# bharath5673/StrongSORT-YOLO

Measured on AMD Instinct MI355X. Metric: tracked frames/sec (whole node), 1280x720@30det, higher is better.
Workload: dtype f32 association / f64 Kalman+LSAP (f16 detector convs, fp32 ReID network on own v_mfma_f32 kernels)

## Files before the change

### strongsort_yolo_amd/csrc/ss_ops.hip

```cpp
#include <hip/hip_fp16.h>
#include <hip/hip_runtime.h>
#include <stdint.h>
#include <stdlib.h>
#include <string>
#include "../../include/strongsort_hip.h"

struct NvEntry { void* stream; const int* n; int batch; };
static thread_local NvEntry g_nv[8] = {};
static inline const int* nv_for(void* stream, long long batch)
{
    for (const NvEntry& e : g_nv) if (e.n && e.stream == stream && e.batch == batch) return e.n;
    return nullptr;
}
static inline int nv_batch(void* stream)
{
    for (const NvEntry& e : g_nv) if (e.n && e.stream == stream) return e.batch;
    return 0;
}

static int g_opt_pw_epilogue = 1, g_opt_pw_splitk = 1, g_opt_osnet_chains = 1;

typedef _Float16 h8 __attribute__((ext_vector_type(8)));
typedef _Float16 h4 __attribute__((ext_vector_type(4)));
typedef float f4 __attribute__((ext_vector_type(4)));

__device__ inline float act_apply(float v, int act)
{
    if (act == 1) return v > 0.f ? v : 0.f;
    if (act == 2) return v * __builtin_amdgcn_rcpf(1.0f + __expf(-v));
    if (act == 3) return __builtin_amdgcn_rcpf(1.0f + __expf(-v));
    return v;
}

__global__ __launch_bounds__(256) void k_bias_act8(__half* __restrict__ x, const __half* __restrict__ bias,
                                                  const __half* __restrict__ res, size_t n_vec, int C8, int act)
{
    for (size_t i = blockIdx.x * (size_t)blockDim.x + threadIdx.x; i < n_vec; i += (size_t)gridDim.x * blockDim.x) {
        h8 v = reinterpret_cast<h8*>(x)[i];
        h8 b = reinterpret_cast<const h8*>(bias)[i % C8];
        h8 r;
        if (res) r = reinterpret_cast<const h8*>(res)[i];
#pragma unroll
        for (int k = 0; k < 8; ++k) {
            float f = (float)v[k] + (float)b[k];
            if (res) f += (float)r[k];
            v[k] = (_Float16)act_apply(f, act);
        }
        reinterpret_cast<h8*>(x)[i] = v;
    }
}

__global__ __launch_bounds__(256) void k_bias_act1(__half* __restrict__ x, const __half* __restrict__ bias,
                                                  const __half* __restrict__ res, size_t n, int C, int act)
{
    for (size_t i = blockIdx.x * (size_t)blockDim.x + threadIdx.x; i < n; i += (size_t)gridDim.x * blockDim.x) {
        float f = __half2float(x[i]) + __half2float(bias[i % C]);
        if (res) f += __half2float(res[i]);
        x[i] = __float2half(act_apply(f, act));
    }
}

__device__ __forceinline__ float ss_mix_lo(unsigned a, unsigned b, float c)
{ float d; asm("v_fma_mix_f32 %0, %1, %2, %3 op_sel:[0,0,0] op_sel_hi:[1,1,0]" : "=v"(d) : "v"(a), "v"(b), "v"(c)); return d; }
__device__ __forceinline__ float ss_mix_hi(unsigned a, unsigned b, float c)
{ float d; asm("v_fma_mix_f32 %0, %1, %2, %3 op_sel:[1,1,0] op_sel_hi:[1,1,0]" : "=v"(d) : "v"(a), "v"(b), "v"(c)); return d; }
__device__ __forceinline__ void ss_dw_tap8(const h8& v, const h8& w, float (&acc)[8])
{
    const uint4 vu = __builtin_bit_cast(uint4, v), wu = __builtin_bit_cast(uint4, w);
    acc[0] = ss_mix_lo(vu.x, wu.x, acc[0]); acc[1] = ss_mix_hi(vu.x, wu.x, acc[1]);
    acc[2] = ss_mix_lo(vu.y, wu.y, acc[2]); acc[3] = ss_mix_hi(vu.y, wu.y, acc[3]);
    acc[4] = ss_mix_lo(vu.z, wu.z, acc[4]); acc[5] = ss_mix_hi(vu.z, wu.z, acc[5]);
    acc[6] = ss_mix_lo(vu.w, wu.w, acc[6]); acc[7] = ss_mix_hi(vu.w, wu.w, acc[7]);
}

__global__ __launch_bounds__(256) void k_dw3x3(const __half* __restrict__ x, const __half* __restrict__ w9,
                                              const __half* __restrict__ bias, __half* __restrict__ y, int N, int H,
                                              int W, int C8, int act)
{
    const size_t total = (size_t)N * H * W * C8;
    for (size_t i = blockIdx.x * (size_t)blockDim.x + threadIdx.x; i < total; i += (size_t)gridDim.x * blockDim.x) {
        const int c8 = (int)(i % C8);
        const size_t p = i / C8;
        const int w = (int)(p % W), h = (int)((p / W) % H);
        const size_t nb = (p / ((size_t)W * H)) * H;
        float acc[8];
        {
            h8 b = reinterpret_cast<const h8*>(bias)[c8];
#pragma unroll
            for (int k = 0; k < 8; ++k) acc[k] = (float)b[k];
        }
#pragma unroll
        for (int dy = -1; dy <= 1; ++dy) {
            const int hh = h + dy;
            if (hh < 0 || hh >= H) continue;
#pragma unroll
            for (int dx = -1; dx <= 1; ++dx) {
                const int ww = w + dx;
                if (ww < 0 || ww >= W) continue;
                h8 v = reinterpret_cast<const h8*>(x)[((nb + hh) * W + ww) * C8 + c8];
                h8 k9 = reinterpret_cast<const h8*>(w9)[((dy + 1) * 3 + dx + 1) * C8 + c8];
                ss_dw_tap8(v, k9, acc);
            }
        }
// ... 332 lines not shown
    f4 acc[MT];
#pragma unroll
    for (int mt = 0; mt < MT; ++mt) acc[mt] = f4{ 0.f, 0.f, 0.f, 0.f };
    h8 a[MT][2], b[2], an[MT][2], bn[2];
    int kc = wave * KC;
    if (kc < K) { load_a(kc, a); load_b(kc, b); }
    for (; kc < K; kc += 4 * KC) {
        const bool more = kc + 4 * KC < K;
        if (more) { load_a(kc + 4 * KC, an); load_b(kc + 4 * KC, bn); }
#pragma unroll
        for (int ks = 0; ks < 2; ++ks) {
            if (kc + ks * 32 >= K) break;
#pragma unroll
            for (int mt = 0; mt < MT; ++mt) acc[mt] = __builtin_amdgcn_mfma_f32_16x16x32_f16(a[mt][ks], b[ks], acc[mt], 0, 0, 0);
        }
        if (more) {
#pragma unroll
            for (int mt = 0; mt < MT; ++mt) { a[mt][0] = an[mt][0]; a[mt][1] = an[mt][1]; }
            b[0] = bn[0]; b[1] = bn[1];
        }
    }
#pragma unroll
    for (int mt = 0; mt < MT; ++mt)
#pragma unroll
        for (int j = 0; j < 4; ++j) Red[(wave * BN + mt * 16 + 4 * q + j) * RP + n] = acc[mt][j];
    __syncthreads();
    constexpr int CG = BN / 8;
    if (tid < 16 * CG) {
        const int row = tid / CG, cg = tid - row * CG;
        const size_t p = (size_t)bx * 16 + row;
        const int oc = n0 + cg * 8;
        if (p < (size_t)M && oc < N) {
            const h8 bb = *reinterpret_cast<const h8*>(bias + oc);
            h8 r = z8;
            if (res) r = *reinterpret_cast<const h8*>(res + p * N + oc);
            h8 o;
#pragma unroll
            for (int j = 0; j < 8; ++j) {
                const int ch = cg * 8 + j;
                const float sum = ((Red[(0 * BN + ch) * RP + row] + Red[(1 * BN + ch) * RP + row]) + Red[(2 * BN + ch) * RP + row]) +
                                  Red[(3 * BN + ch) * RP + row];
                float f = (float)(_Float16)sum + (float)bb[j];
                if (res && !res_after) f += (float)r[j];
                f = act_apply(f, act);
                if (res && res_after) f = (float)(_Float16)f + (float)r[j];
                o[j] = (_Float16)f;
            }
            *reinterpret_cast<h8*>(out + p * out_ld + oc) = o;
            if (out2 && oc >= c0 && oc < c0 + cn) *reinterpret_cast<h8*>(out2 + p * cn + (oc - c0)) = o;
        }
    }
}

template <int BN, bool CONV3>
__global__ __launch_bounds__(256) void k_pw_splitk(PwArgs A) { pw_splitk_body<BN, CONV3>(A, blockIdx.x, blockIdx.y); }

#define PW_GROUP_MAX 12
struct PwGroup { PwArgs p[PW_GROUP_MAX]; int start[PW_GROUP_MAX + 1]; int form[PW_GROUP_MAX]; int n; };

#ifndef SS_GRP_WAVES
#define SS_GRP_WAVES 6
#endif
template <int BN, bool CONV3, bool SPLITK>
__global__ __launch_bounds__(256)
__attribute__((amdgpu_waves_per_eu(SPLITK || !SS_GRP_WAVES ? 1 : SS_GRP_WAVES)))
void k_pw_group(PwGroup G)
{
    __shared__ __attribute__((aligned(16))) _Float16 pw_lds[pw_lds_halfs<BN, 1, true>()];
    int bx = blockIdx.x, p = 0;
    for (int i = 1; i < G.n; ++i) if (bx >= G.start[i]) p = i;
    bx -= G.start[p];
    const int form = G.form[p];
    if constexpr (SPLITK) { if (form == 1) { pw_splitk_body<BN, CONV3>(G.p[p], bx, 0); return; } }
    if (BN == 80 && G.p[p].N <= 64) pw_body<64, 1, CONV3, true>(G.p[p], bx, 0, pw_lds);
    else pw_body<BN, 1, CONV3, true>(G.p[p], bx, 0, pw_lds);
}

struct BnArgs {
    const __half* x; const __half* w1; const __half* b1; const __half* w2; const __half* b2;
    __half* out; int out_ld; __half* out2;
    int B, H, W, add, TW, TH, tiles_x, tiles_y;
};

template <int CI, int CO, int PT>
__device__ __forceinline__ void bn_conv(const _Float16* __restrict__ In, const int (&pbase)[PT], const int* __restrict__ tapoff,
                                        const __half* __restrict__ w, _Float16* __restrict__ Ws, f4 (&acc)[CO / 16][PT], const int tid)
{
    constexpr int C = CI;
    constexpr int MT = CO / 16, WP = 72, K = 9 * CI, WV = (CO * 8 + 255) / 256;
    const int lane = tid & 63, q = lane >> 4, n = lane & 15;
    const h8 z8 = { 0, 0, 0, 0, 0, 0, 0, 0 };
    auto load_w = [&](int k0, h8 (&wr)[WV]) {
#pragma unroll
        for (int j = 0; j < WV; ++j) {
            const int i = tid + j * 256, r = i >> 3, c8 = i & 7, kk = k0 + c8 * 8;
            wr[j] = (i < CO * 8 && kk < K) ? *reinterpret_cast<const h8*>(w + (size_t)r * K + kk) : z8;
        }
    };
    h8 wr[WV], wn[WV];
    load_w(0, wr);
    int buf = 0;
    for (int k0 = 0; k0 < K; k0 += 64, buf ^= 1) {
        _Float16* wb = Ws + buf * (CO * WP);
#pragma unroll
        for (int j = 0; j < WV; ++j) {
            const int i = tid + j * 256, r = i >> 3, c8 = i & 7;
            if (i < CO * 8) *reinterpret_cast<h8*>(wb + r * WP + c8 * 8) = wr[j];
        }
        if (k0 + 64 < K) load_w(k0 + 64, wn);
        __syncthreads();
        h8 b[2][PT], a[2][MT];
#pragma unroll
        for (int ks = 0; ks < 2; ++ks) {
            const int kk = k0 + ks * 32 + 8 * q, tap = kk / C, c = kk % C;
            const bool kv = kk < K;
            const int boff = kv ? tapoff[tap] + c : 0;
#pragma unroll
            for (int pt = 0; pt < PT; ++pt) {
                b[ks][pt] = *reinterpret_cast<const h8*>(In + pbase[pt] + boff);
                if (!kv) b[ks][pt] = z8;
            }
#pragma unroll
            for (int mt = 0; mt < MT; ++mt) a[ks][mt] = *reinterpret_cast<const h8*>(wb + (mt * 16 + n) * WP + ks * 32 + 8 * q);
        }
#pragma unroll
        for (int ks = 0; ks < 2; ++ks) {
            if (k0 + ks * 32 >= K) break;
#pragma unroll
            for (int mt = 0; mt < MT; ++mt)
#pragma unroll
                for (int pt = 0; pt < PT; ++pt)
                    acc[mt][pt] = __builtin_amdgcn_mfma_f32_16x16x32_f16(a[ks][mt], b[ks][pt], acc[mt][pt], 0, 0, 0);
        }
        if (k0 + 64 < K) {
#pragma unroll
            for (int j = 0; j < WV; ++j) wr[j] = wn[j];
        }
    }
}

template <int C, int PT1, int PT2>
__global__ __launch_bounds__(256) __attribute__((amdgpu_waves_per_eu(!SS_TAIL_BUMP ? 1 : C == 16 ? 6 : 1))) void k_bneck(BnArgs A)
{
    extern __shared__ __attribute__((aligned(16))) char bn_smem[];
    constexpr int MT = C / 16, P = C + 8, WP = 72;
    const int tid = threadIdx.x, lane = tid & 63, wave = tid >> 6, q = lane >> 4, n = lane & 15;
    const int TW = A.TW, TH = A.TH, XW = TW + 4, XH = TH + 4, RW = TW + 2, RH = TH + 2;
    _Float16* Xs = reinterpret_cast<_Float16*>(bn_smem);
    _Float16* Ts = Xs + XH * XW * P;
    _Float16* Ws = Ts + ((RH * RW * P + 7) & ~7);
    int* tap1 = reinterpret_cast<int*>(Ws + 2 * C * WP);
    int* tap2 = tap1 + 16;
    const int tpi = A.tiles_x * A.tiles_y;
    const int img = blockIdx.x / tpi, trm = blockIdx.x - img * tpi, tyi = trm / A.tiles_x, txi = trm - tyi * A.tiles_x;
    const int oy0 = tyi * TH, ox0 = txi * TW, H = A.H, W = A.W;
    const h8 z8 = { 0, 0, 0, 0, 0, 0, 0, 0 };
    if (tid < 9) { const int ky = tid / 3, kx = tid - ky * 3; tap1[tid] = (ky * XW + kx) * P; tap2[tid] = (ky * RW + kx) * P; }
    const __half* xi = A.x + (size_t)img * H * W * C;
    constexpr int VPC = C / 8;
    const int rowv = XW * VPC;
    for (int r = wave; r < XH; r += 4) {
        const int iy = oy0 - 2 + r;
        const bool rok = iy >= 0 && iy < H;
        const __half* src = xi + (size_t)(rok ? iy : 0) * W * C;
        _Float16* dst = Xs + r * XW * P;
        for (int i0 = lane; i0 < rowv; i0 += 512) {
            h8 tmp[8];
#pragma unroll
            for (int u = 0; u < 8; ++u) {
                const int i = i0 + 64 * u, c = i / VPC, v = i % VPC, ix = ox0 - 2 + c;
                const bool ok = rok && i < rowv && ix >= 0 && ix < W;
                tmp[u] = ok ? *reinterpret_cast<const h8*>(src + (size_t)ix * C + v * 8) : z8;
            }
#pragma unroll
            for (int u = 0; u < 8; ++u) {
                const int i = i0 + 64 * u, c = i / VPC, v = i % VPC;
                if (i < rowv) *reinterpret_cast<h8*>(dst + c * P + v * 8) = tmp[u];
            }
        }
    }
    {
        int pb[PT1], tpix[PT1];
        bool inimg[PT1];
#pragma unroll
        for (int pt = 0; pt < PT1; ++pt) {
            const int p = (wave * PT1 + pt) * 16 + n;
            int ry = p / RW, rx = p - ry * RW;
            const bool ok = p < RH * RW;
            if (!ok) { ry = 0; rx = 0; }
            const int iy = oy0 - 1 + ry, ix = ox0 - 1 + rx;
            inimg[pt] = ok && iy >= 0 && iy < H && ix >= 0 && ix < W;
            tpix[pt] = ok ? p : -1;
            pb[pt] = (ry * XW + rx) * P;
        }
        f4 acc[MT][PT1];
#pragma unroll
        for (int mt = 0; mt < MT; ++mt)
#pragma unroll
            for (int pt = 0; pt < PT1; ++pt) acc[mt][pt] = f4{ 0.f, 0.f, 0.f, 0.f };
        bn_conv<C, C, PT1>(Xs, pb, tap1, A.w1, Ws, acc, tid);
#pragma unroll
        for (int mt = 0; mt < MT; ++mt) {
            const h4 bb = *reinterpret_cast<const h4*>(A.b1 + mt * 16 + 4 * q);
#pragma unroll
            for (int pt = 0; pt < PT1; ++pt) {
                if (tpix[pt] < 0) continue;
                h4 o;
#pragma unroll
                for (int j = 0; j < 4; ++j) {
                    float f = act_apply((float)(_Float16)acc[mt][pt][j] + (float)bb[j], 2);
                    asm volatile("" : "+v"(f));
                    o[j] = inimg[pt] ? (_Float16)f : (_Float16)0.f;
                }
                *reinterpret_cast<h4*>(Ts + tpix[pt] * P + mt * 16 + 4 * q) = o;
            }
        }
    }
    __syncthreads();
    {
        int pb[PT2], opix[PT2], xoff[PT2];
#pragma unroll
        for (int pt = 0; pt < PT2; ++pt) {
            const int p = (wave * PT2 + pt) * 16 + n;
            int ty = p / TW, tx = p - ty * TW;
            const bool ok = p < TH * TW && oy0 + ty < H && ox0 + tx < W;
            if (!ok) { ty = 0; tx = 0; }
            pb[pt] = (ty * RW + tx) * P;
            xoff[pt] = ((ty + 2) * XW + tx + 2) * P;
            opix[pt] = ok ? (img * H + oy0 + ty) * W + ox0 + tx : -1;
        }
        f4 acc[MT][PT2];
#pragma unroll
        for (int mt = 0; mt < MT; ++mt)
#pragma unroll
            for (int pt = 0; pt < PT2; ++pt) acc[mt][pt] = f4{ 0.f, 0.f, 0.f, 0.f };
        bn_conv<C, C, PT2>(Ts, pb, tap2, A.w2, Ws, acc, tid);
#pragma unroll
        for (int mt = 0; mt < MT; ++mt) {
            const h4 bb = *reinterpret_cast<const h4*>(A.b2 + mt * 16 + 4 * q);
#pragma unroll
            for (int pt = 0; pt < PT2; ++pt) {
                if (opix[pt] < 0) continue;
                const h4 xr = *reinterpret_cast<const h4*>(Xs + xoff[pt] + mt * 16 + 4 * q);
                h4 o;
#pragma unroll
                for (int j = 0; j < 4; ++j) {
                    float f = act_apply((float)(_Float16)acc[mt][pt][j] + (float)bb[j], 2);
                    asm volatile("" : "+v"(f));
                    if (A.add) f = (float)(_Float16)f + (float)xr[j];
                    o[j] = (_Float16)f;
                }
                *reinterpret_cast<h4*>(A.out + (size_t)opix[pt] * A.out_ld + mt * 16 + 4 * q) = o;
                if (A.out2) *reinterpret_cast<h4*>(A.out2 + (size_t)opix[pt] * C + mt * 16 + 4 * q) = o;
            }
        }
    }
}

struct HeadArgs {
    const __half* x;
    const __half* w1[2]; const __half* b1[2]; const __half* w2[2]; const __half* b2[2]; const __half* w3[2]; const __half* b3[2];
    __half* out[2]; int nout[2];
    int B, H, W, TW, TH, tiles_x, tiles_y;
};

template <int CI, int CM, int PT1, int PT2>
__device__ __forceinline__ void head_body(const HeadArgs& A, const int br, char* smem)
{
    constexpr int MT = CM / 16, PX = CI + 8, PM = CM + 8, WP = 72, KB3 = (CM + 31) / 32;
    const int tid = threadIdx.x, lane = tid & 63, wave = tid >> 6, q = lane >> 4, n = lane & 15;
    const int TW = A.TW, TH = A.TH, XW = TW + 4, XH = TH + 4, RW = TW + 2, RH = TH + 2;
    _Float16* Xs = reinterpret_cast<_Float16*>(smem);
    _Float16* Ts = Xs + ((XH * XW * PX + 7) & ~7);
    _Float16* Ws = Ts + ((RH * RW * PM + 7) & ~7);
    int* tap1 = reinterpret_cast<int*>(Ws + 2 * 80 * WP);
    int* tap2 = tap1 + 16;
    _Float16* Us = Xs;
    const int tpi = A.tiles_x * A.tiles_y;
    const int img = blockIdx.x / tpi, trm = blockIdx.x - img * tpi, tyi = trm / A.tiles_x, txi = trm - tyi * A.tiles_x;
    const int oy0 = tyi * TH, ox0 = txi * TW, H = A.H, W = A.W;
    const h8 z8 = { 0, 0, 0, 0, 0, 0, 0, 0 };
    if (tid < 9) { const int ky = tid / 3, kx = tid - ky * 3; tap1[tid] = (ky * XW + kx) * PX; tap2[tid] = (ky * RW + kx) * PM; }
    const __half* xi = A.x + (size_t)img * H * W * CI;
    constexpr int VPC = CI / 8;
    const int rowv = XW * VPC;
    for (int r = wave; r < XH; r += 4) {
        const int iy = oy0 - 2 + r;
        const bool rok = iy >= 0 && iy < H;
        const __half* src = xi + (size_t)(rok ? iy : 0) * W * CI;
        _Float16* dst = Xs + r * XW * PX;
        for (int i0 = lane; i0 < rowv; i0 += 512) {
            h8 tmp[8];
#pragma unroll
            for (int u = 0; u < 8; ++u) {
                const int i = i0 + 64 * u, c = i / VPC, v = i % VPC, ix = ox0 - 2 + c;
                const bool ok = rok && i < rowv && ix >= 0 && ix < W;
                tmp[u] = ok ? *reinterpret_cast<const h8*>(src + (size_t)ix * CI + v * 8) : z8;
            }
#pragma unroll
            for (int u = 0; u < 8; ++u) {
                const int i = i0 + 64 * u, c = i / VPC, v = i % VPC;
                if (i < rowv) *reinterpret_cast<h8*>(dst + c * PX + v * 8) = tmp[u];
            }
        }
    }
    {
        int pb[PT1], tpix[PT1];
        bool inimg[PT1];
#pragma unroll
        for (int pt = 0; pt < PT1; ++pt) {
            const int p = (wave * PT1 + pt) * 16 + n;
            int ry = p / RW, rx = p - ry * RW;
            const bool ok = p < RH * RW;
            if (!ok) { ry = 0; rx = 0; }
            const int iy = oy0 - 1 + ry, ix = ox0 - 1 + rx;
            inimg[pt] = ok && iy >= 0 && iy < H && ix >= 0 && ix < W;
            tpix[pt] = ok ? p : -1;
            pb[pt] = (ry * XW + rx) * PX;
        }
        f4 acc[MT][PT1];
#pragma unroll
        for (int mt = 0; mt < MT; ++mt)
#pragma unroll
            for (int pt = 0; pt < PT1; ++pt) acc[mt][pt] = f4{ 0.f, 0.f, 0.f, 0.f };
        bn_conv<CI, CM, PT1>(Xs, pb, tap1, A.w1[br], Ws, acc, tid);
#pragma unroll
        for (int mt = 0; mt < MT; ++mt) {
            const h4 bb = *reinterpret_cast<const h4*>(A.b1[br] + mt * 16 + 4 * q);
#pragma unroll
            for (int pt = 0; pt < PT1; ++pt) {
                if (tpix[pt] < 0) continue;
                h4 o;
#pragma unroll
                for (int j = 0; j < 4; ++j) {
                    float f = act_apply((float)(_Float16)acc[mt][pt][j] + (float)bb[j], 2);
                    asm volatile("" : "+v"(f));
                    o[j] = inimg[pt] ? (_Float16)f : (_Float16)0.f;
                }
// ... 1761 lines not shown
        if (c.N > nmax) nmax = c.N;
        order[i] = i;
        cost[i] = (long long)c.ksize * c.ksize * c.Cin;
    }
    for (int i = 1; i < n; ++i)
        for (int j = i; j > 0 && cost[order[j]] > cost[order[j - 1]]; --j) { const int t = order[j]; order[j] = order[j - 1]; order[j - 1] = t; }
    int wgs = 0;
    for (int s = 0; s < n; ++s) {
        const ss_conv_desc& c = d[order[s]];
        ConvGeom g{ c.H, c.W, c.Cin, (c.H - 1) / c.stride + 1, (c.W - 1) / c.stride + 1, c.stride };
        const long long M = (long long)c.B * g.OH * g.OW;
        if (M > 0x7fffffffLL) return SS_ERR_INVALID;
        const int K = c.ksize * c.ksize * c.Cin;
        G.p[s] = PwArgs{ (const __half*)c.x, (const __half*)c.w, (const __half*)c.bias, nullptr, (int)M, K, c.N, c.act, 0, (__half*)c.out,
                         c.N, nullptr, 0, 0, g, nullptr, 0 };
        G.form[s] = (splitk_allowed && conv3 && K >= 512 && M <= 4096) ? 1 : 0;
        G.start[s] = wgs;
        wgs += (int)(G.form[s] == 1 ? (M + 15) / 16 : (M + 63) / 64);
    }
    for (int s = n; s < PW_GROUP_MAX; ++s) { G.p[s] = G.p[0]; G.form[s] = 0; G.start[s] = wgs; }
    G.start[PW_GROUP_MAX] = wgs;
    G.n = n;
    hipStream_t st = (hipStream_t)stream;
    bool any_splitk = false;
    for (int s = 0; s < n; ++s) any_splitk = any_splitk || G.form[s] == 1;
#define SS_GRP(BN) do { if (conv3 && any_splitk) hipLaunchKernelGGL((k_pw_group<BN, true, true>), dim3(wgs), dim3(256), 0, st, G);            \
                        else if (conv3) hipLaunchKernelGGL((k_pw_group<BN, true, false>), dim3(wgs), dim3(256), 0, st, G);                    \
                        else hipLaunchKernelGGL((k_pw_group<BN, false, false>), dim3(wgs), dim3(256), 0, st, G); } while (0)
    if (nmax <= 32) SS_GRP(32);
    else if (nmax <= 64) SS_GRP(64);
    else SS_GRP(80);
#undef SS_GRP
    return hipGetLastError() == hipSuccess ? SS_OK : SS_ERR_HIP;
}

extern "C" int ss_op_upcat_f16(void* stream, const void* lo, const void* hi, void* out, int B, int h, int w, int C1, int C2, int lo_first)
{
    if (!lo || !hi || !out || B < 1 || h < 1 || w < 1 || C1 < 8 || C1 % 8 || C2 < 8 || C2 % 8) return SS_ERR_INVALID;
    const size_t total = (size_t)B * 4 * h * w * ((C1 + C2) / 8);
    hipLaunchKernelGGL(k_upcat, dim3(grid_for(total, 256)), dim3(256), 0, (hipStream_t)stream, (const __half*)lo, (const __half*)hi,
                       (__half*)out, B, h, w, C1 / 8, C2 / 8, lo_first);
    return hipGetLastError() == hipSuccess ? SS_OK : SS_ERR_HIP;
}

extern "C" int ss_op_osnet_head_f16(void* stream, const void* x, const void* w, const void* bias, void* out, int N, int HW, int C, int F)
{
    if (!x || !w || !bias || !out || N < 1 || HW < 1 || C != 128 || F < 1) return SS_ERR_INVALID;
    hipLaunchKernelGGL(k_osnet_head<128>, dim3((N + 3) / 4), dim3(256), 0, (hipStream_t)stream, (const __half*)x, (const __half*)w,
                       (const __half*)bias, (__half*)out, N, HW, F, nv_for(stream, N));
    return hipGetLastError() == hipSuccess ? SS_OK : SS_ERR_HIP;
}

extern "C" int ss_op_psa_attention_f16(void* stream, const void* qkv, const void* pe, void* out, int B, int N, int heads, float scale)
{
    if (!qkv || !out || B < 1 || B > 65535 || N < 1 || N > 16 * PSA_MAXT || heads < 1 || heads > 64) return SS_ERR_INVALID;
    const int NP = (N + 31) & ~31;
    hipLaunchKernelGGL(k_psa_attn, dim3((N + 63) / 64, heads, B), dim3(256), (size_t)64 * (NP + 16) * 2, (hipStream_t)stream,
                       (const __half*)qkv, (const __half*)pe, (__half*)out, N, heads, scale);
    return hipGetLastError() == hipSuccess ? SS_OK : SS_ERR_HIP;
}

extern "C" int ss_op_sppf_pools_f16(void* stream, const void* x, void* out, int B, int H, int W, int C)
{
    if (!x || !out || B < 1 || H < 1 || W < 1 || C < 8 || C % 8 || H * W > 1024) return SS_ERR_INVALID;
    hipLaunchKernelGGL(k_sppf_pools, dim3((unsigned)(B * (C / 8))), dim3(256), (size_t)2 * H * W * 16, (hipStream_t)stream,
                       (const __half*)x, (__half*)out, H, W, C / 8);
    return hipGetLastError() == hipSuccess ? SS_OK : SS_ERR_HIP;
}

extern "C" int ss_op_conv0_f16(void* stream, const void* x, const void* w_prep, const void* bias, void* y, int B, int H, int W, int Cout,
                               int act)
{
    if (!x || !w_prep || !bias || !y || B < 1 || H < 2 || W < 128 || W % 128 || (W * 3) % 8 || (Cout != 16 && Cout != 32 && Cout != 48))
        return SS_ERR_INVALID;
    const int OH = (H - 1) / 2 + 1;
    const dim3 grid(W / 128, (OH + C0_ROWS - 1) / C0_ROWS, B), block(256);
    hipStream_t st = (hipStream_t)stream;
#define SS_C0(CO) hipLaunchKernelGGL(k_conv0<CO>, grid, block, 0, st, (const __half*)x, (const __half*)w_prep, (const __half*)bias, (__half*)y, H, W, act)
    if (Cout == 16) SS_C0(16); else if (Cout == 32) SS_C0(32); else SS_C0(48);
#undef SS_C0
    return hipGetLastError() == hipSuccess ? SS_OK : SS_ERR_HIP;
}

extern "C" int ss_op_bottleneck_f16(void* stream, const void* x, const void* w1, const void* b1, const void* w2, const void* b2, int B, int H,
                                    int W, int C, int add, void* out, int out_ld, void* out2)
{
    if (!x || !w1 || !b1 || !w2 || !b2 || !out || B < 1 || H < 1 || W < 1 || (C != 16 && C != 32 && C != 64 && C != 128) || out_ld < C || out_ld % 4 ||
        ((uintptr_t)out % 8) || ((uintptr_t)x % 16) || ((uintptr_t)w1 % 16) || ((uintptr_t)w2 % 16) || (out2 && ((uintptr_t)out2 % 8)))
        return SS_ERR_INVALID;
    const long long M = (long long)B * H * W;
    const bool big = M / 128 >= 512 && C <= 64;
    BnArgs A{ (const __half*)x, (const __half*)w1, (const __half*)b1, (const __half*)w2, (const __half*)b2, (__half*)out, out_ld, (__half*)out2,
              B, H, W, add, big ? 16 : 8, 8, 0, 0 };
    A.tiles_x = (W + A.TW - 1) / A.TW; A.tiles_y = (H + A.TH - 1) / A.TH;
    const int P = C + 8;
    const size_t lds = ((size_t)(A.TH + 4) * (A.TW + 4) * P + (((size_t)(A.TH + 2) * (A.TW + 2) * P + 7) & ~(size_t)7) + 2 * (size_t)C * 72) * 2 + 128;
    const dim3 grid((unsigned)(B * A.tiles_x * A.tiles_y));
    hipStream_t st = (hipStream_t)stream;
#define SS_BN(CC, P1, P2) do { static unsigned long long attr = 0; int dv_ = 0; (void)hipGetDevice(&dv_); if (!(attr >> (dv_ & 63) & 1)) { (void)hipFuncSetAttribute((const void*)k_bneck<CC, P1, P2>, hipFuncAttributeMaxDynamicSharedMemorySize, 160 * 1024 - 512); attr |= 1ull << (dv_ & 63); }    \
                               hipLaunchKernelGGL((k_bneck<CC, P1, P2>), grid, dim3(256), lds, st, A); } while (0)
    if (big) { if (C == 16) SS_BN(16, 3, 2); else if (C == 32) SS_BN(32, 3, 2); else SS_BN(64, 3, 2); }
    else { if (C == 16) SS_BN(16, 2, 1); else if (C == 32) SS_BN(32, 2, 1); else if (C == 64) SS_BN(64, 2, 1); else SS_BN(128, 2, 1); }
#undef SS_BN
    return hipGetLastError() == hipSuccess ? SS_OK : SS_ERR_HIP;
}

extern "C" int ss_op_head_f16(void* stream, const void* x, const void* const* w1, const void* const* b1, const void* const* w2,
                              const void* const* b2, const void* const* w3, const void* const* b3, void* const* out, const int* nout,
                              int B, int H, int W, int Cin, int tile16)
{
    if (!x || !w1 || !b1 || !w2 || !b2 || !w3 || !b3 || !out || !nout || B < 1 || H < 1 || W < 1 || (Cin != 64 && Cin != 128 && Cin != 256) ||
        ((uintptr_t)x % 16))
        return SS_ERR_INVALID;
    HeadArgs A;
    A.x = (const __half*)x;
    for (int b = 0; b < 2; ++b) {
        const int cm = b ? 80 : 64;
        if (!w1[b] || !b1[b] || !w2[b] || !b2[b] || !w3[b] || !b3[b] || !out[b] || nout[b] < 8 || nout[b] % 8 || nout[b] > cm ||
            ((uintptr_t)w1[b] % 16) || ((uintptr_t)w2[b] % 16) || ((uintptr_t)w3[b] % 16) || ((uintptr_t)out[b] % 8))
            return SS_ERR_INVALID;
        A.w1[b] = (const __half*)w1[b]; A.b1[b] = (const __half*)b1[b]; A.w2[b] = (const __half*)w2[b]; A.b2[b] = (const __half*)b2[b];
        A.w3[b] = (const __half*)w3[b]; A.b3[b] = (const __half*)b3[b]; A.out[b] = (__half*)out[b]; A.nout[b] = nout[b];
    }
    const bool big = tile16 != 0 && Cin == 64;
    A.B = B; A.H = H; A.W = W; A.TW = big ? 16 : 8; A.TH = 8;
    A.tiles_x = (W + A.TW - 1) / A.TW; A.tiles_y = (H + A.TH - 1) / A.TH;
    const size_t xs = ((size_t)(A.TH + 4) * (A.TW + 4) * (Cin + 8) + 7) & ~(size_t)7, ts = ((size_t)(A.TH + 2) * (A.TW + 2) * 88 + 7) & ~(size_t)7;
    const size_t lds = (xs + ts + 2 * 80 * 72) * 2 + 128;
    if (lds > 160 * 1024 - 512) return SS_ERR_INVALID;
    const dim3 grid((unsigned)(B * A.tiles_x * A.tiles_y), 2);
    hipStream_t st = (hipStream_t)stream;
#define SS_HD(CC, P1, P2) do { static unsigned long long attr = 0; int dv_ = 0; (void)hipGetDevice(&dv_); if (!(attr >> (dv_ & 63) & 1)) { (void)hipFuncSetAttribute((const void*)k_head<CC, P1, P2>, hipFuncAttributeMaxDynamicSharedMemorySize, 160 * 1024 - 512); attr |= 1ull << (dv_ & 63); }    \
                               hipLaunchKernelGGL((k_head<CC, P1, P2>), grid, dim3(256), lds, st, A); } while (0)
    if (big) SS_HD(64, 3, 2);
    else if (Cin == 64) SS_HD(64, 2, 1);
    else if (Cin == 128) SS_HD(128, 2, 1);
    else SS_HD(256, 2, 1);
#undef SS_HD
    return hipGetLastError() == hipSuccess ? SS_OK : SS_ERR_HIP;
}

extern "C" int ss_op_set_valid_images(void* stream, const int* d_n, int batch)
{
    NvEntry* slot = nullptr;
    for (NvEntry& e : g_nv) if (e.n && e.stream == stream) slot = &e;
    if (!d_n) { if (slot) *slot = NvEntry{}; return SS_OK; }
    if (batch < 1) return SS_ERR_INVALID;
    if (!slot) for (NvEntry& e : g_nv) if (!e.n) { slot = &e; break; }
    if (!slot) return SS_ERR_CAPACITY;
    *slot = NvEntry{ stream, d_n, batch };
    return SS_OK;
}

extern int g_opt_jpeg_subseq_words;
int ss_aflink_chunk_option(int value);
extern "C" int ss_op_set_option(const char* name, int value)
{
    if (!name) return SS_ERR_INVALID;
    const std::string n(name);
    if (n == "pw_epilogue") g_opt_pw_epilogue = value;
    else if (n == "pw_splitk") g_opt_pw_splitk = value;
    else if (n == "osnet_chains") g_opt_osnet_chains = value;
    else if (n == "jpeg_subseq_words") { if (value != 4 && value != 8 && value != 16 && value != 32) return SS_ERR_INVALID; g_opt_jpeg_subseq_words = value; }
    else if (n == "aflink_chunk") return ss_aflink_chunk_option(value);
    else return SS_ERR_INVALID;
    return SS_OK;
}
```

Measured before the change: 8615.

## Add persistent bottleneck kernel keeping both conv weights resident in LDS

Result: slower. 8478 (-1.6%).

```diff
diff --git a/strongsort_yolo_amd/csrc/ss_ops.hip b/strongsort_yolo_amd/csrc/ss_ops.hip
--- a/strongsort_yolo_amd/csrc/ss_ops.hip
+++ b/strongsort_yolo_amd/csrc/ss_ops.hip
@@ -19,6 +19,7 @@
 }
 
 static int g_opt_pw_epilogue = 1, g_opt_pw_splitk = 1, g_opt_osnet_chains = 1;
+static int g_opt_bneck_resident = 1;
 
 typedef _Float16 h8 __attribute__((ext_vector_type(8)));
 typedef _Float16 h4 __attribute__((ext_vector_type(4)));
@@ -517,11 +518,41 @@
     int B, H, W, add, TW, TH, tiles_x, tiles_y;
 };
 
+template <int C, int MT, int PT>
+__device__ __forceinline__ void bn_slice(const _Float16* __restrict__ In, const int (&pbase)[PT], const int* __restrict__ tapoff,
+                                         const _Float16* __restrict__ wl, const int wmt, const int k0, const int q, f4 (&acc)[MT][PT])
+{
+    constexpr int K = 9 * C;
+    const h8 z8 = { 0, 0, 0, 0, 0, 0, 0, 0 };
+    h8 b[2][PT], a[2][MT];
+#pragma unroll
+    for (int ks = 0; ks < 2; ++ks) {
+        const int kk = k0 + ks * 32 + 8 * q, tap = kk / C, c = kk % C;
+        const bool kv = kk < K;
+        const int boff = kv ? tapoff[tap] + c : 0;
+#pragma unroll
+        for (int pt = 0; pt < PT; ++pt) {
+            b[ks][pt] = *reinterpret_cast<const h8*>(In + pbase[pt] + boff);
+            if (!kv) b[ks][pt] = z8;
+        }
+#pragma unroll
+        for (int mt = 0; mt < MT; ++mt) a[ks][mt] = *reinterpret_cast<const h8*>(wl + mt * wmt + ks * 32);
+    }
+#pragma unroll
+    for (int ks = 0; ks < 2; ++ks) {
+        if (k0 + ks * 32 >= K) break;
+#pragma unroll
+        for (int mt = 0; mt < MT; ++mt)
+#pragma unroll
+            for (int pt = 0; pt < PT; ++pt)
+                acc[mt][pt] = __builtin_amdgcn_mfma_f32_16x16x32_f16(a[ks][mt], b[ks][pt], acc[mt][pt], 0, 0, 0);
+    }
+}
+
 template <int CI, int CO, int PT>
 __device__ __forceinline__ void bn_conv(const _Float16* __restrict__ In, const int (&pbase)[PT], const int* __restrict__ tapoff,
                                         const __half* __restrict__ w, _Float16* __restrict__ Ws, f4 (&acc)[CO / 16][PT], const int tid)
 {
-    constexpr int C = CI;
     constexpr int MT = CO / 16, WP = 72, K = 9 * CI, WV = (CO * 8 + 255) / 256;
     const int lane = tid & 63, q = lane >> 4, n = lane & 15;
     const h8 z8 = { 0, 0, 0, 0, 0, 0, 0, 0 };
@@ -544,32 +575,59 @@
         }
         if (k0 + 64 < K) load_w(k0 + 64, wn);
         __syncthreads();
-        h8 b[2][PT], a[2][MT];
-#pragma unroll
-        for (int ks = 0; ks < 2; ++ks) {
-            const int kk = k0 + ks * 32 + 8 * q, tap = kk / C, c = kk % C;
-            const bool kv = kk < K;
-            const int boff = kv ? tapoff[tap] + c : 0;
-#pragma unroll
-            for (int pt = 0; pt < PT; ++pt) {
-                b[ks][pt] = *reinterpret_cast<const h8*>(In + pbase[pt] + boff);
-                if (!kv) b[ks][pt] = z8;
-            }
-#pragma unroll
-            for (int mt = 0; mt < MT; ++mt) a[ks][mt] = *reinterpret_cast<const h8*>(wb + (mt * 16 + n) * WP + ks * 32 + 8 * q);
-        }
-#pragma unroll
-        for (int ks = 0; ks < 2; ++ks) {
-            if (k0 + ks * 32 >= K) break;
-#pragma unroll
-            for (int mt = 0; mt < MT; ++mt)
-#pragma unroll
-                for (int pt = 0; pt < PT; ++pt)
-                    acc[mt][pt] = __builtin_amdgcn_mfma_f32_16x16x32_f16(a[ks][mt], b[ks][pt], acc[mt][pt], 0, 0, 0);
-        }
+        bn_slice<CI, MT, PT>(In, pbase, tapoff, wb + n * WP + 8 * q, 16 * WP, k0, q, acc);
         if (k0 + 64 < K) {
 #pragma unroll
             for (int j = 0; j < WV; ++j) wr[j] = wn[j];
+        }
+    }
+}
+
+template <int C, int PT>
+__device__ __forceinline__ void bn_mid_epilogue(const f4 (&acc)[C / 16][PT], const _Float16* __restrict__ bias, const int (&tpix)[PT],
+                                                const bool (&inimg)[PT], _Float16* __restrict__ Ts, const int q)
+{
+    constexpr int MT = C / 16, P = C + 8;
+#pragma unroll
+    for (int mt = 0; mt < MT; ++mt) {
+        const h4 bb = *reinterpret_cast<const h4*>(bias + mt * 16 + 4 * q);
+#pragma unroll
+        for (int pt = 0; pt < PT; ++pt) {
+            if (tpix[pt] < 0) continue;
+            h4 o;
+#pragma unroll
+            for (int j = 0; j < 4; ++j) {
+                float f = act_apply((float)(_Float16)acc[mt][pt][j] + (float)bb[j], 2);
+                asm volatile("" : "+v"(f));
+                o[j] = inimg[pt] ? (_Float16)f : (_Float16)0.f;
+            }
+            *reinterpret_cast<h4*>(Ts + tpix[pt] * P + mt * 16 + 4 * q) = o;
+        }
+    }
+}
+
+template <int C, int PT>
+__device__ __forceinline__ void bn_out_epilogue(const f4 (&acc)[C / 16][PT], const _Float16* __restrict__ bias, const int (&opix)[PT],
+                                                const int (&xoff)[PT], const _Float16* __restrict__ Xs, const BnArgs& A, const int q)
+{
+    constexpr int MT = C / 16;
+#pragma unroll
+    for (int mt = 0; mt < MT; ++mt) {
+        const h4 bb = *reinterpret_cast<const h4*>(bias + mt * 16 + 4 * q);
+#pragma unroll
+        for (int pt = 0; pt < PT; ++pt) {
+            if (opix[pt] < 0) continue;
+            const h4 xr = *reinterpret_cast<const h4*>(Xs + xoff[pt] + mt * 16 + 4 * q);
+            h4 o;
+#pragma unroll
+            for (int j = 0; j < 4; ++j) {
+                float f = act_apply((float)(_Float16)acc[mt][pt][j] + (float)bb[j], 2);
+                asm volatile("" : "+v"(f));
+                if (A.add) f = (float)(_Float16)f + (float)xr[j];
+                o[j] = (_Float16)f;
+            }
+            *reinterpret_cast<h4*>(A.out + (size_t)opix[pt] * A.out_ld + mt * 16 + 4 * q) = o;
+            if (A.out2) *reinterpret_cast<h4*>(A.out2 + (size_t)opix[pt] * C + mt * 16 + 4 * q) = o;
         }
     }
 }
@@ -634,22 +692,7 @@
 #pragma unroll
             for (int pt = 0; pt < PT1; ++pt) acc[mt][pt] = f4{ 0.f, 0.f, 0.f, 0.f };
         bn_conv<C, C, PT1>(Xs, pb, tap1, A.w1, Ws, acc, tid);
-#pragma unroll
-        for (int mt = 0; mt < MT; ++mt) {
-            const h4 bb = *reinterpret_cast<const h4*>(A.b1 + mt * 16 + 4 * q);
-#pragma unroll
-            for (int pt = 0; pt < PT1; ++pt) {
-                if (tpix[pt] < 0) continue;
-                h4 o;
-#pragma unroll
-                for (int j = 0; j < 4; ++j) {
-                    float f = act_apply((float)(_Float16)acc[mt][pt][j] + (float)bb[j], 2);
-                    asm volatile("" : "+v"(f));
-                    o[j] = inimg[pt] ? (_Float16)f : (_Float16)0.f;
-                }
-                *reinterpret_cast<h4*>(Ts + tpix[pt] * P + mt * 16 + 4 * q) = o;
-            }
-        }
+        bn_mid_epilogue<C, PT1>(acc, reinterpret_cast<const _Float16*>(A.b1), tpix, inimg, Ts, q);
     }
     __syncthreads();
     {
@@ -670,25 +713,153 @@
 #pragma unroll
             for (int pt = 0; pt < PT2; ++pt) acc[mt][pt] = f4{ 0.f, 0.f, 0.f, 0.f };
         bn_conv<C, C, PT2>(Ts, pb, tap2, A.w2, Ws, acc, tid);
-#pragma unroll
-        for (int mt = 0; mt < MT; ++mt) {
-            const h4 bb = *reinterpret_cast<const h4*>(A.b2 + mt * 16 + 4 * q);
+        bn_out_epilogue<C, PT2>(acc, reinterpret_cast<const _Float16*>(A.b2), opix, xoff, Xs, A, q);
+    }
+}
+
+template <int C> constexpr int bnr_pitch() { return C == 16 ? 176 : 304; }
+template <int C> constexpr size_t bnr_lds_bytes()
+{
+    return ((size_t)12 * 20 * (C + 8) + ((10 * 18 * (C + 8) + 7) & ~7) + 2 * C * bnr_pitch<C>() + 2 * C) * 2 + 128;
+}
+
+template <int CI, int CO, int PT, int WR>
+__device__ __forceinline__ void bn_conv_res(const _Float16* __restrict__ In, const int (&pbase)[PT], const int* __restrict__ tapoff,
+                                            const _Float16* __restrict__ Wm, f4 (&acc)[CO / 16][PT], const int tid)
+{
+    constexpr int K = 9 * CI;
+    const int lane = tid & 63, q = lane >> 4, n = lane & 15;
+#pragma unroll
+    for (int k0 = 0; k0 < K; k0 += 64)
+        bn_slice<CI, CO / 16, PT>(In, pbase, tapoff, Wm + n * WR + k0 + 8 * q, 16 * WR, k0, q, acc);
+}
+
+template <int C>
+__global__ __launch_bounds__(256) __attribute__((amdgpu_waves_per_eu(C == 16 ? 5 : 2))) void k_bneck_res(BnArgs A)
+{
+    extern __shared__ __attribute__((aligned(16))) char bn_smem[];
+    constexpr int MT = C / 16, P = C + 8, K = 9 * C, KV = K / 8, WR = bnr_pitch<C>(), PADV = (WR - K) / 8, PT1 = 3, PT2 = 2;
+    constexpr int TW = 16, TH = 8, XW = TW + 4, XH = TH + 4, RW = TW + 2, RH = TH + 2, VPC = C / 8;
+    constexpr int NX = XH * XW * VPC, XV = (NX + 255) / 256;
+    constexpr int NW = 2 * C * KV, WV = (NW + 255) / 256;
+    static_assert(RH * RW <= 4 * PT1 * 16 && TH * TW == 4 * PT2 * 16 && (WR / 8) % 4 == 2 && WR >= K, "tile / pitch");
+    const int tid = threadIdx.x, lane = tid & 63, wave = tid >> 6, q = lane >> 4, n = lane & 15;
+    const int H = A.H, W = A.W, tpi = A.tiles_x * A.tiles_y, ntiles = A.B * tpi, G = gridDim.x;
+    int t = blockIdx.x;
+    if (t >= ntiles) return;
+    _Float16* Xs = reinterpret_cast<_Float16*>(bn_smem);
+    _Float16* Ts = Xs + XH * XW * P;
+    _Float16* W1s = Ts + ((RH * RW * P + 7) & ~7);
+    _Float16* W2s = W1s + C * WR;
+    _Float16* Bs = W2s + C * WR;
+    int* tap1 = reinterpret_cast<int*>(Bs + 2 * C);
+    int* tap2 = tap1 + 16;
+    const h8 z8 = { 0, 0, 0, 0, 0, 0, 0, 0 };
+    if (tid < 9) { const int ky = tid / 3, kx = tid - ky * 3; tap1[tid] = (ky * XW + kx) * P; tap2[tid] = (ky * RW + kx) * P; }
+    int img = 0, oy0 = 0, ox0 = 0;
+    auto tile_at = [&](int tile, int& ti, int& ty0, int& tx0) {
+        ti = tile / tpi;
+        const int trm = tile - ti * tpi, tyi = trm / A.tiles_x;
+        ty0 = tyi * TH; tx0 = (trm - tyi * A.tiles_x) * TW;
+    };
+    h8 xv[XV];
+    auto load_x = [&](int tile) {
+        int ti, ty0, tx0;
+        tile_at(tile, ti, ty0, tx0);
+        const __half* xi = A.x + (size_t)ti * H * W * C;
+#pragma unroll
+        for (int j = 0; j < XV; ++j) {
+            const int i = tid + j * 256, px = i / VPC, v = i % VPC, r = px / XW, c = px - r * XW, iy = ty0 - 2 + r, ix = tx0 - 2 + c;
+            const bool ok = i < NX && iy >= 0 && iy < H && ix >= 0 && ix < W;
+            xv[j] = ok ? *reinterpret_cast<const h8*>(xi + ((size_t)iy * W + ix) * C + v * 8) : z8;
+        }
+    };
+    {
+        h8 wv[WV];
+#pragma unroll
+        for (int j = 0; j < WV; ++j) {
+            const int i = tid + j * 256, m = i / (C * KV), rr = i - m * (C * KV);
+            wv[j] = i < NW ? *reinterpret_cast<const h8*>((m ? A.w2 : A.w1) + (size_t)rr * 8) : z8;
+        }
+        h4 bv = { 0, 0, 0, 0 };
+        if (tid < 2 * C / 4) bv = *reinterpret_cast<const h4*>((tid < C / 4 ? A.b1 : A.b2) + (tid % (C / 4)) * 4);
+        load_x(t);
+#pragma unroll
+        for (int j = 0; j < WV; ++j) {
+            const int i = tid + j * 256, row = i / KV, c8 = i - row * KV;
+            if (i < NW) *reinterpret_cast<h8*>(W1s + row * WR + c8 * 8) = wv[j];
+        }
+        if (tid < 2 * C / 4) *reinterpret_cast<h4*>(Bs + tid * 4) = bv;
+        for (int i = tid; i < 2 * C * PADV; i += 256) {
+            const int row = i / PADV, c8 = i - row * PADV;
+            *reinterpret_cast<h8*>(W1s + row * WR + K + c8 * 8) = z8;
+        }
+    }
+    int pb1[PT1], tp1[PT1], ry1[PT1], rx1[PT1];
+#pragma unroll
+    for (int pt = 0; pt < PT1; ++pt) {
+        const int p = (wave * PT1 + pt) * 16 + n;
+        int ry = p / RW, rx = p - ry * RW;
+        const bool ok = p < RH * RW;
+        if (!ok) { ry = 0; rx = 0; }
+        tp1[pt] = ok ? p : -1; ry1[pt] = ry; rx1[pt] = rx;
+        pb1[pt] = (ry * XW + rx) * P;
+    }
+    int pb2[PT2], xoff[PT2], ty2[PT2], tx2[PT2];
+#pragma unroll
+    for (int pt = 0; pt < PT2; ++pt) {
+        const int p = (wave * PT2 + pt) * 16 + n, ty = p / TW, tx = p - ty * TW;
+        ty2[pt] = ty; tx2[pt] = tx;
+        pb2[pt] = (ty * RW + tx) * P;
+        xoff[pt] = ((ty + 2) * XW + tx + 2) * P;
+    }
+    for (;;) {
+#pragma unroll
+        for (int j = 0; j < XV; ++j) {
+            const int i = tid + j * 256, px = i / VPC, v = i % VPC;
+            if (i < NX) *reinterpret_cast<h8*>(Xs + px * P + v * 8) = xv[j];
+        }
+        __syncthreads();
+        tile_at(t, img, oy0, ox0);
+        const int tn = t + G;
+        const bool more = tn < ntiles;
+        if (more) load_x(tn);
+        {
+            int tpix[PT1];
+            bool inimg[PT1];
+#pragma unroll
+            for (int pt = 0; pt < PT1; ++pt) {
+                const int iy = oy0 - 1 + ry1[pt], ix = ox0 - 1 + rx1[pt];
+                tpix[pt] = tp1[pt];
+                inimg[pt] = tp1[pt] >= 0 && iy >= 0 && iy < H && ix >= 0 && ix < W;
+            }
+            f4 acc[MT][PT1];
+#pragma unroll
+            for (int mt = 0; mt < MT; ++mt)
+#pragma unroll
+                for (int pt = 0; pt < PT1; ++pt) acc[mt][pt] = f4{ 0.f, 0.f, 0.f, 0.f };
+            bn_conv_res<C, C, PT1, WR>(Xs, pb1, tap1, W1s, acc, tid);
+            bn_mid_epilogue<C, PT1>(acc, Bs, tpix, inimg, Ts, q);
+        }
+        __syncthreads();
+        {
+            int opix[PT2];
 #pragma unroll
             for (int pt = 0; pt < PT2; ++pt) {
-                if (opix[pt] < 0) continue;
-                const h4 xr = *reinterpret_cast<const h4*>(Xs + xoff[pt] + mt * 16 + 4 * q);
-                h4 o;
-#pragma unroll
-                for (int j = 0; j < 4; ++j) {
-                    float f = act_apply((float)(_Float16)acc[mt][pt][j] + (float)bb[j], 2);
-                    asm volatile("" : "+v"(f));
-                    if (A.add) f = (float)(_Float16)f + (float)xr[j];
-                    o[j] = (_Float16)f;
-                }
-                *reinterpret_cast<h4*>(A.out + (size_t)opix[pt] * A.out_ld + mt * 16 + 4 * q) = o;
-                if (A.out2) *reinterpret_cast<h4*>(A.out2 + (size_t)opix[pt] * C + mt * 16 + 4 * q) = o;
-            }
-        }
+                const int oy = oy0 + ty2[pt], ox = ox0 + tx2[pt];
+                opix[pt] = (oy < H && ox < W) ? (img * H + oy) * W + ox : -1;
+            }
+            f4 acc[MT][PT2];
+#pragma unroll
+            for (int mt = 0; mt < MT; ++mt)
+#pragma unroll
+                for (int pt = 0; pt < PT2; ++pt) acc[mt][pt] = f4{ 0.f, 0.f, 0.f, 0.f };
+            bn_conv_res<C, C, PT2, WR>(Ts, pb2, tap2, W2s, acc, tid);
+            bn_out_epilogue<C, PT2>(acc, Bs + C, opix, xoff, Xs, A, q);
+        }
+        if (!more) break;
+        __syncthreads();
+        t = tn;
     }
 }
 
@@ -2616,12 +2787,48 @@
     return hipGetLastError() == hipSuccess ? SS_OK : SS_ERR_HIP;
 }
 
+template <int C> static int bnr_full_grid()
+{
+    static int full[64] = {};
+    static unsigned long long known = 0;
+    int dv = 0;
+    (void)hipGetDevice(&dv);
+    dv &= 63;
+    if (!(known >> dv & 1)) {
+        int occ = 0, cus = 0;
+        (void)hipFuncSetAttribute((const void*)k_bneck_res<C>, hipFuncAttributeMaxDynamicSharedMemorySize, 160 * 1024 - 512);
+        if (hipOccupancyMaxActiveBlocksPerMultiprocessor(&occ, k_bneck_res<C>, 256, bnr_lds_bytes<C>()) != hipSuccess ||
+            hipDeviceGetAttribute(&cus, hipDeviceAttributeMultiprocessorCount, dv) != hipSuccess) {
+            (void)hipGetLastError();
+            occ = 0;
+        }
+        full[dv] = occ * cus;
+        known |= 1ull << dv;
+    }
+    return full[dv];
+}
+
 extern "C" int ss_op_bottleneck_f16(void* stream, const void* x, const void* w1, const void* b1, const void* w2, const void* b2, int B, int H,
                                     int W, int C, int add, void* out, int out_ld, void* out2)
 {
     if (!x || !w1 || !b1 || !w2 || !b2 || !out || B < 1 || H < 1 || W < 1 || (C != 16 && C != 32 && C != 64 && C != 128) || out_ld < C || out_ld % 4 ||
         ((uintptr_t)out % 8) || ((uintptr_t)x % 16) || ((uintptr_t)w1 % 16) || ((uintptr_t)w2 % 16) || (out2 && ((uintptr_t)out2 % 8)))
         return SS_ERR_INVALID;
+    hipStream_t st = (hipStream_t)stream;
+    if ((C == 16 || C == 32) && g_opt_bneck_resident != 0) {
+        BnArgs A{ (const __half*)x, (const __half*)w1, (const __half*)b1, (const __half*)w2, (const __half*)b2, (__half*)out, out_ld, (__half*)out2,
+                  B, H, W, add, 16, 8, (W + 15) / 16, (H + 7) / 8 };
+        const long long ntiles = (long long)B * A.tiles_x * A.tiles_y;
+        const int full = C == 16 ? bnr_full_grid<16>() : bnr_full_grid<32>();
+        long long G = 0;
+        if (g_opt_bneck_resident < 0) G = -(long long)g_opt_bneck_resident;
+        else if (full > 0 && 2 * ntiles >= 3 * (long long)full) G = full;
+        if (G > 0 && ntiles <= 0x7fffffff) {
+            if (C == 16) hipLaunchKernelGGL(k_bneck_res<16>, dim3((unsigned)G), dim3(256), bnr_lds_bytes<16>(), st, A);
+            else hipLaunchKernelGGL(k_bneck_res<32>, dim3((unsigned)G), dim3(256), bnr_lds_bytes<32>(), st, A);
+            return hipGetLastError() == hipSuccess ? SS_OK : SS_ERR_HIP;
+        }
+    }
     const long long M = (long long)B * H * W;
     const bool big = M / 128 >= 512 && C <= 64;
     BnArgs A{ (const __half*)x, (const __half*)w1, (const __half*)b1, (const __half*)w2, (const __half*)b2, (__half*)out, out_ld, (__half*)out2,
@@ -2630,7 +2837,6 @@
     const int P = C + 8;
     const size_t lds = ((size_t)(A.TH + 4) * (A.TW + 4) * P + (((size_t)(A.TH + 2) * (A.TW + 2) * P + 7) & ~(size_t)7) + 2 * (size_t)C * 72) * 2 + 128;
     const dim3 grid((unsigned)(B * A.tiles_x * A.tiles_y));
-    hipStream_t st = (hipStream_t)stream;
 #define SS_BN(CC, P1, P2) do { static unsigned long long attr = 0; int dv_ = 0; (void)hipGetDevice(&dv_); if (!(attr >> (dv_ & 63) & 1)) { (void)hipFuncSetAttribute((const void*)k_bneck<CC, P1, P2>, hipFuncAttributeMaxDynamicSharedMemorySize, 160 * 1024 - 512); attr |= 1ull << (dv_ & 63); }    \
                                hipLaunchKernelGGL((k_bneck<CC, P1, P2>), grid, dim3(256), lds, st, A); } while (0)
     if (big) { if (C == 16) SS_BN(16, 3, 2); else if (C == 32) SS_BN(32, 3, 2); else SS_BN(64, 3, 2); }
@@ -2695,6 +2901,7 @@
     if (n == "pw_epilogue") g_opt_pw_epilogue = value;
     else if (n == "pw_splitk") g_opt_pw_splitk = value;
     else if (n == "osnet_chains") g_opt_osnet_chains = value;
+    else if (n == "bneck_resident") { if (value > 1 || value < -65536) return SS_ERR_INVALID; g_opt_bneck_resident = value; }
     else if (n == "jpeg_subseq_words") { if (value != 4 && value != 8 && value != 16 && value != 32) return SS_ERR_INVALID; g_opt_jpeg_subseq_words = value; }
     else if (n == "aflink_chunk") return ss_aflink_chunk_option(value);
     else return SS_ERR_INVALID;
```
